# jnvance/DMRG.x

Measured on AMD Instinct MI355X. Metric: superblock MatMults/sec inside the ground-state eigensolve (Lanczos step = 1 MatMult + reorthogonalisation), higher is better.
Workload: dtype f64

## Files before the change

### dmrg.x_amd/csrc/eigs.hip

```cpp
#include "common.h"
#include <mutex>
#include <algorithm>
#include <chrono>
#include <cmath>
#include <cstring>
#include <cstddef>

namespace dmrgx {
namespace {

constexpr int DOT_BLOCKS = 1024, DOT_THREADS = 256, DOT_CHUNK = 8, MAX_NCV = 64, FUSE_NV = 24, GD_NV = 8;

__device__ __forceinline__ double wave_sum(double v) {
#pragma unroll
    for (int o = 32; o > 0; o >>= 1) v += __shfl_down(v, o, 64);
    return v;
}

template <bool VEC2>
__global__ void __launch_bounds__(DOT_THREADS)
multi_dot_kernel(const double* __restrict__ V, int64_t ldv, int nv, const double* __restrict__ w, int64_t n, double* __restrict__ partial)
{
    __shared__ double red[DOT_THREADS / 64][DOT_CHUNK];
    const int v0 = blockIdx.y * DOT_CHUNK;
    double acc[DOT_CHUNK];
#pragma unroll
    for (int i = 0; i < DOT_CHUNK; ++i) acc[i] = 0.0;
    if (VEC2) {
        const double2* __restrict__ w2 = reinterpret_cast<const double2*>(w);
        for (int64_t e = (int64_t)blockIdx.x * DOT_THREADS + threadIdx.x; e < n / 2; e += (int64_t)gridDim.x * DOT_THREADS) {
            const double2 wv = w2[e];
#pragma unroll
            for (int i = 0; i < DOT_CHUNK; ++i) {
                const int v = v0 + i;
                if (v < nv) { const double2 x = reinterpret_cast<const double2*>(V + (int64_t)v * ldv)[e]; acc[i] += x.x * wv.x + x.y * wv.y; }
                else if (v == nv) acc[i] += wv.x * wv.x + wv.y * wv.y;
            }
        }
    } else {
        for (int64_t e = (int64_t)blockIdx.x * DOT_THREADS + threadIdx.x; e < n; e += (int64_t)gridDim.x * DOT_THREADS) {
            const double wv = w[e];
#pragma unroll
            for (int i = 0; i < DOT_CHUNK; ++i) {
                const int v = v0 + i;
                if (v < nv) acc[i] += V[(int64_t)v * ldv + e] * wv;
                else if (v == nv) acc[i] += wv * wv;
            }
        }
    }
    const int lane = threadIdx.x & 63, wave = threadIdx.x >> 6;
#pragma unroll
    for (int i = 0; i < DOT_CHUNK; ++i) {
        const double s = wave_sum(acc[i]);
        if (lane == 0) red[wave][i] = s;
    }
    __syncthreads();
    if (threadIdx.x < DOT_CHUNK) {
        double s = 0.0;
        for (int wv = 0; wv < DOT_THREADS / 64; ++wv) s += red[wv][threadIdx.x];
        partial[(int64_t)(v0 + threadIdx.x) * gridDim.x + blockIdx.x] = s;
    }
}

__global__ void __launch_bounds__(DOT_THREADS)
reduce_partials_kernel(const double* __restrict__ partial, double* __restrict__ out, int count, int nblk)
{
    __shared__ double red[DOT_THREADS / 64];
    const int i = blockIdx.x;
    if (i >= count) return;
    double s = 0.0;
    for (int b = threadIdx.x; b < nblk; b += DOT_THREADS) s += partial[(int64_t)i * nblk + b];
    s = wave_sum(s);
    if ((threadIdx.x & 63) == 0) red[threadIdx.x >> 6] = s;
    __syncthreads();
    if (threadIdx.x == 0) { double t = 0.0; for (int k = 0; k < DOT_THREADS / 64; ++k) t += red[k]; out[i] = t; }
}

__global__ void __launch_bounds__(DOT_THREADS)
multi_axpy_kernel(const double* __restrict__ V, int64_t ldv, int nv, const double* __restrict__ c, double* __restrict__ w, int64_t n,
                  double* __restrict__ partial, double* __restrict__ hacc)
{
    __shared__ double cs[MAX_NCV + 1];
    __shared__ double red[DOT_THREADS / 64];
    if (threadIdx.x < nv) cs[threadIdx.x] = c[threadIdx.x];
    __syncthreads();
    if (blockIdx.x == 0 && threadIdx.x < nv && hacc) hacc[threadIdx.x] += cs[threadIdx.x];
    double nrm = 0.0;
    for (int64_t e = (int64_t)blockIdx.x * DOT_THREADS + threadIdx.x; e < n; e += (int64_t)gridDim.x * DOT_THREADS) {
        double x = w[e];
        for (int i = 0; i < nv; ++i) x -= cs[i] * V[(int64_t)i * ldv + e];
        w[e] = x;
        nrm += x * x;
    }
    nrm = wave_sum(nrm);
    if ((threadIdx.x & 63) == 0) red[threadIdx.x >> 6] = nrm;
    __syncthreads();
    if (threadIdx.x == 0) { double t = 0.0; for (int k = 0; k < DOT_THREADS / 64; ++k) t += red[k]; partial[blockIdx.x] = t; }
}

template <int NVMAX>
__global__ void __launch_bounds__(DOT_THREADS)
axpy_dot_kernel(const double* __restrict__ V, int64_t ldv, int nv, const double* __restrict__ c, double* __restrict__ w, int64_t n,
                double* __restrict__ partial, double* __restrict__ hacc)
{
    __shared__ double cs[NVMAX];
    __shared__ double red[DOT_THREADS / 64][NVMAX + 1];
    if (threadIdx.x < nv) cs[threadIdx.x] = c[threadIdx.x];
    __syncthreads();
    if (blockIdx.x == 0 && threadIdx.x < nv && hacc) hacc[threadIdx.x] += cs[threadIdx.x];
    double acc[NVMAX + 1];
#pragma unroll
    for (int i = 0; i <= NVMAX; ++i) acc[i] = 0.0;
    for (int64_t e = (int64_t)blockIdx.x * DOT_THREADS + threadIdx.x; e < n; e += (int64_t)gridDim.x * DOT_THREADS) {
        double v[NVMAX];
#pragma unroll
        for (int i = 0; i < NVMAX; ++i) v[i] = i < nv ? V[(int64_t)i * ldv + e] : 0.0;
        double x = w[e];
#pragma unroll
        for (int i = 0; i < NVMAX; ++i) if (i < nv) x -= cs[i] * v[i];
        w[e] = x;
#pragma unroll
        for (int i = 0; i < NVMAX; ++i) if (i < nv) acc[i] += v[i] * x;
        acc[NVMAX] += x * x;
    }
    const int lane = threadIdx.x & 63, wave = threadIdx.x >> 6;
#pragma unroll
    for (int i = 0; i <= NVMAX; ++i) {
        if (i < nv || i == NVMAX) {
            const double s2 = wave_sum(acc[i]);
            if (lane == 0) red[wave][i] = s2;
        }
    }
    __syncthreads();
    if (threadIdx.x <= nv) {
        const int src = threadIdx.x < nv ? threadIdx.x : NVMAX;
        double s2 = 0.0;
        for (int wv = 0; wv < DOT_THREADS / 64; ++wv) s2 += red[wv][src];
        partial[(int64_t)threadIdx.x * gridDim.x + blockIdx.x] = s2;
    }
}

template <bool VEC2>
__global__ void __launch_bounds__(DOT_THREADS)
axpy_normalise_kernel(const double* __restrict__ V, int64_t ldv, int nv, const double* __restrict__ c, const double* __restrict__ w,
                      double* __restrict__ dst, int64_t n, double* __restrict__ beta2_out, double* __restrict__ hacc)
{
    __shared__ double cs[MAX_NCV + 2];
    if (threadIdx.x <= nv) cs[threadIdx.x] = c[threadIdx.x];
    __syncthreads();
    if (blockIdx.x == 0 && threadIdx.x < nv && hacc) hacc[threadIdx.x] += cs[threadIdx.x];
    double s2 = cs[nv], sc = 0.0;
    for (int i = 0; i < nv; ++i) { s2 -= cs[i] * cs[i]; sc += cs[i] * cs[i]; }
    s2 = s2 > 0.0 ? s2 : 0.0;
    if (blockIdx.x == 0 && threadIdx.x == 0 && beta2_out) *beta2_out = s2;
    const double inv = s2 > 1e-290 ? 1.0 / sqrt(s2) : 0.0;
    if (sc <= 1e-27 * cs[nv]) nv = 0;
    if (VEC2) {
        const double2* __restrict__ w2 = reinterpret_cast<const double2*>(w);
        double2* __restrict__ d2 = reinterpret_cast<double2*>(dst);
        for (int64_t e = (int64_t)blockIdx.x * DOT_THREADS + threadIdx.x; e < n / 2; e += (int64_t)gridDim.x * DOT_THREADS) {
            double2 x = w2[e];
            for (int i = 0; i < nv; ++i) { const double2 v = reinterpret_cast<const double2*>(V + (int64_t)i * ldv)[e]; x.x -= cs[i] * v.x; x.y -= cs[i] * v.y; }
            x.x *= inv; x.y *= inv;
            d2[e] = x;
        }
    } else {
        for (int64_t e = (int64_t)blockIdx.x * DOT_THREADS + threadIdx.x; e < n; e += (int64_t)gridDim.x * DOT_THREADS) {
            double x = w[e];
            for (int i = 0; i < nv; ++i) x -= cs[i] * V[(int64_t)i * ldv + e];
            dst[e] = x * inv;
        }
    }
}

__global__ void norm_after_projection_kernel(const double* __restrict__ c, int nv, double* __restrict__ nrm2)
{
    if (threadIdx.x == 0 && blockIdx.x == 0) { double s = c[nv]; for (int i = 0; i < nv; ++i) s -= c[i] * c[i]; *nrm2 = s > 0.0 ? s : 0.0; }
}

__global__ void scale_copy_kernel(const double* __restrict__ src, double* __restrict__ dst, int64_t n, const double* __restrict__ nrm2)
{
    const double s2 = *nrm2;
    const double inv = s2 > 1e-290 ? 1.0 / sqrt(s2) : 0.0;
    for (int64_t e = (int64_t)blockIdx.x * blockDim.x + threadIdx.x; e < n; e += (int64_t)gridDim.x * blockDim.x) dst[e] = src[e] * inv;
}

__global__ void __launch_bounds__(DOT_THREADS)
basis_rotate_kernel(const double* __restrict__ V, int64_t ldv, int m, const double* __restrict__ Q, int ldq, int k,
                    double* __restrict__ out, int64_t ldo, int64_t n)
{
    __shared__ double qs[MAX_NCV * DOT_CHUNK];
    const int j0 = blockIdx.y * DOT_CHUNK;
    for (int t = threadIdx.x; t < m * DOT_CHUNK; t += DOT_THREADS) {
        const int i = t / DOT_CHUNK, j = t % DOT_CHUNK;
        qs[t] = (j0 + j < k) ? Q[i * ldq + j0 + j] : 0.0;
    }
    __syncthreads();
    for (int64_t e = (int64_t)blockIdx.x * DOT_THREADS + threadIdx.x; e < n; e += (int64_t)gridDim.x * DOT_THREADS) {
        double acc[DOT_CHUNK];
#pragma unroll
        for (int j = 0; j < DOT_CHUNK; ++j) acc[j] = 0.0;
        for (int i = 0; i < m; ++i) {
            const double v = V[(int64_t)i * ldv + e];
#pragma unroll
            for (int j = 0; j < DOT_CHUNK; ++j) acc[j] += v * qs[i * DOT_CHUNK + j];
        }
#pragma unroll
        for (int j = 0; j < DOT_CHUNK; ++j) if (j0 + j < k) out[(int64_t)(j0 + j) * ldo + e] = acc[j];
    }
}

constexpr int GD_MAX = FUSE_NV;
constexpr int GD_LD = GD_MAX;
struct GdState {
    double G[GD_MAX * GD_LD];
    double Y[GD_MAX * GD_LD];
    double th[GD_MAX];
    double y[GD_MAX];
    double yprev[GD_MAX];
    double Q[GD_MAX * GD_LD];
    double theta;
    double hv0_2;
    double e0[GD_MAX];
    int after_restart;
    int pad_;
};

constexpr int RITZ_THREADS = 64;
__global__ void __launch_bounds__(RITZ_THREADS)
gd_ritz_kernel(GdState* __restrict__ S, const double* __restrict__ col_src, int col_is_partial, int nblk, int mm, int warm, int restart, int keep)
{
    __shared__ double A[GD_MAX][GD_MAX + 1], Qa[GD_MAX][GD_MAX + 1], Yn[GD_MAX][GD_MAX + 1], Yp[GD_MAX][GD_MAX + 1];
    __shared__ double col[GD_MAX + 1], cs_c[GD_MAX / 2], cs_s[GD_MAX / 2], dg[GD_MAX], thp[GD_MAX], ths[GD_MAX];
    __shared__ int pp[GD_MAX / 2], qq[GD_MAX / 2], perm[GD_MAX];
    __shared__ double offn, dgn;
    const int tid = threadIdx.x, lane = tid;
    const int j = mm - 1;
    if (warm && mm > 1) {
        for (int e = tid; e < (mm - 1) * (mm - 1); e += RITZ_THREADS) Yp[e / (mm - 1)][e % (mm - 1)] = S->Y[(e / (mm - 1)) * GD_LD + e % (mm - 1)];
        if (tid < mm - 1) thp[tid] = S->th[tid];
    }
    const double yold = tid < GD_MAX ? S->y[tid] : 0.0;
    const int was_restart = S->after_restart;
// ... 346 lines not shown
    static thread_local double* p = nullptr;
    if (!p && hipHostMalloc((void**)&p, (8 + MAX_NCV + 2) * sizeof(double), hipHostMallocDefault) != hipSuccess) { (void)hipGetLastError(); p = nullptr; }
    return p;
}
static bool start_too_light(const dmrgx_eigs_opts* opts, const double* pin)
{
    return opts->min_initial_norm2 > 0.0 && pin && !(pin[2] >= opts->min_initial_norm2);
}

extern "C" dmrgx_status dmrgx_eigs_lowest(dmrgx_kron_plan* plan, const dmrgx_eigs_opts* opts, double* e0,
                                          double* psi_full, dmrgx_eigs_stats* stats, void* stream)
{
    hipStream_t st = (hipStream_t)stream;
    if (!plan || !opts || !e0 || !psi_full) DMRGX_FAIL(DMRGX_ERR_ARG, "eigs_lowest: null argument");
    dmrgx_kron_info I;
    DMRGX_CHK(dmrgx_kron_plan_info(plan, &I));
    const bool gd_space = std::min<int64_t>(opts->ncv > 0 ? opts->ncv : 16, I.n_states) >= 2;
    if (opts->method == 1 && opts->use_initial && opts->max_matvec <= 0 && gd_space) return eigs_davidson(plan, opts, e0, psi_full, stats, st);
    const bool dist = I.vec_len != I.n_states;
    const bool hooks = opts->allgather && opts->allreduce_sum;
    if (dist && !hooks && !opts->comm) DMRGX_FAIL(DMRGX_ERR_ARG, "eigs_lowest: a striped plan needs a communicator (opts->comm) or the allgather/allreduce hooks");
    auto gather_full = [&](double* full) -> dmrgx_status {
        return hooks ? opts->allgather(opts->user, full, I.seg_stride, st) : dmrgx_comm_allgather(opts->comm, full, I.seg_stride, st);
    };
    const int64_t n = I.local_len, N = I.n_states;
    int m = opts->ncv > 0 ? opts->ncv : 16;
    m = (int)std::min<int64_t>(std::min(m, MAX_NCV), N);
    m = (int)std::max<int64_t>(m, std::min<int64_t>(2, N));
    if (m < 1) DMRGX_FAIL(DMRGX_ERR_ARG, "eigs_lowest: empty problem");
    const int max_it = opts->max_it > 0 ? opts->max_it : std::max<int>(100, (int)(2 * N / m));
    const double tol = opts->tol > 0 ? opts->tol : 1e-8;
    const auto t_begin = std::chrono::steady_clock::now();

    DevBuf dV, dW, dX, dTmp, dPartial, dScal, dQ;
    DMRGX_CHK(dV.alloc_f64((size_t)(m + 1) * n, st));
    DMRGX_CHK(dW.alloc_f64((size_t)n, st));
    DMRGX_CHK(dTmp.alloc_f64((size_t)(m / 2 + 2) * n, st));
    if (dist) DMRGX_CHK(dX.alloc_f64((size_t)I.vec_len, st));
    DMRGX_CHK(dPartial.alloc_f64((size_t)(MAX_NCV + DOT_CHUNK + 1) * DOT_BLOCKS, st));
    const int row = m + 2;
    DMRGX_CHK(dScal.alloc_f64((size_t)((m + 1) * row + 3 * (MAX_NCV + 2)), st));
    DMRGX_CHK(dQ.alloc_f64((size_t)MAX_NCV * MAX_NCV, st));
    double* V = dV.as<double>();
    double* w = dW.as<double>();
    double* c1 = dScal.as<double>() + (size_t)(m + 1) * row;
    double* c2 = c1 + (MAX_NCV + 2);
    double* nrm = c2 + (MAX_NCV + 2);
    auto Hrow = [&](int j) { return dScal.as<double>() + (size_t)j * row; };
    auto vec = [&](int j) { return V + (size_t)j * n; };
    DMRGX_HIP(zero_async(dV.p, dV.bytes, st));
    DMRGX_HIP(zero_async(dW.p, dW.bytes, st));
    if (dist) DMRGX_HIP(zero_async(dX.p, dX.bytes, st));

    const bool vec2 = (n % 2 == 0);
    const int nblk = DOT_BLOCKS;
    auto allreduce = [&](double* buf, int64_t count) -> dmrgx_status {
        if (!dist) return DMRGX_OK;
        return hooks ? opts->allreduce_sum(opts->user, buf, count, st) : dmrgx_comm_allreduce_sum(opts->comm, buf, count, st);
    };
    auto multi_dot = [&](int nv) -> dmrgx_status {
        const int chunks = (nv + 1 + DOT_CHUNK - 1) / DOT_CHUNK;
        if (vec2) hipLaunchKernelGGL(multi_dot_kernel<true>, dim3(nblk, chunks), dim3(DOT_THREADS), 0, st, V, n, nv, w, n, dPartial.as<double>());
        else hipLaunchKernelGGL(multi_dot_kernel<false>, dim3(nblk, chunks), dim3(DOT_THREADS), 0, st, V, n, nv, w, n, dPartial.as<double>());
        DMRGX_HIP(hipGetLastError());
        hipLaunchKernelGGL(reduce_partials_kernel, dim3(nv + 1), dim3(DOT_THREADS), 0, st, dPartial.as<double>(), c1, nv + 1, nblk);
        DMRGX_HIP(hipGetLastError());
        return allreduce(c1, nv + 1);
    };
    auto multi_axpy = [&](int nv, double* hacc, bool final) -> dmrgx_status {
        if (final) { hipLaunchKernelGGL(norm_after_projection_kernel, dim3(1), dim3(64), 0, st, c1, nv, nrm); DMRGX_HIP(hipGetLastError()); }
        hipLaunchKernelGGL(multi_axpy_kernel, dim3(nblk), dim3(DOT_THREADS), 0, st, V, n, nv, c1, w, n, dPartial.as<double>(), hacc);
        DMRGX_HIP(hipGetLastError());
        return DMRGX_OK;
    };
    auto normalise_into = [&](double* dst) -> dmrgx_status {
        hipLaunchKernelGGL(scale_copy_kernel, dim3(1024), dim3(256), 0, st, w, dst, n, nrm);
        DMRGX_HIP(hipGetLastError());
        return DMRGX_OK;
    };
    CommTimer ctimer(st);
    auto matvec = [&](const double* v_local, double* y_local) -> dmrgx_status {
        if (!dist) return dmrgx_kron_apply(plan, v_local, y_local, st);
        DMRGX_HIP(hipMemcpyAsync(dX.as<double>() + I.local_offset, v_local, (size_t)n * sizeof(double), hipMemcpyDeviceToDevice, st));
        ctimer.mark();
        DMRGX_CHK(gather_full(dX.as<double>()));
        ctimer.mark();
        const dmrgx_status rc = dmrgx_kron_apply(plan, dX.as<double>(), y_local, st);
        ctimer.mark();
        return rc;
    };

    if (opts->use_initial) DMRGX_HIP(hipMemcpyAsync(w, psi_full + I.local_offset, (size_t)n * sizeof(double), hipMemcpyDeviceToDevice, st));
    else {
        if (!dist) { hipLaunchKernelGGL(random_fill_kernel, dim3(1024), dim3(256), 0, st, w, n, opts->seed, (int64_t)0); DMRGX_HIP(hipGetLastError()); }
        else {
            DevBuf ref;
            DMRGX_CHK(ref.alloc((size_t)N * sizeof(double)));
            hipLaunchKernelGGL(random_fill_kernel, dim3(1024), dim3(256), 0, st, ref.as<double>(), N, opts->seed, (int64_t)0);
            DMRGX_HIP(hipGetLastError());
            DMRGX_CHK(dmrgx_kron_vec_to_striped(plan, ref.as<double>(), dX.as<double>(), st));
            DMRGX_HIP(hipMemcpyAsync(w, dX.as<double>() + I.local_offset, (size_t)n * sizeof(double), hipMemcpyDeviceToDevice, st));
            DMRGX_HIP(hipStreamSynchronize(st));
        }
    }
// ... 10 lines not shown
    if (looks && !look_buf) {
        DMRGX_HIP(hipHostMalloc((void**)&look_buf, 2 * look_stride * sizeof(double), hipHostMallocDefault));
        DMRGX_HIP(hipEventCreateWithFlags(&look_ev[0], hipEventDisableTiming)); DMRGX_HIP(hipEventCreateWithFlags(&look_ev[1], hipEventDisableTiming));
    }
    int look_mm[2] = {0, 0};
    std::vector<double> T((size_t)m * m, 0.0), theta, Q, hbuf((size_t)(m + 1) * row);
    int k = 0, n_matvec = 0, restarts = 0, converged = 0;
    double beta_m = 0.0, resid = 0.0, lambda = 0.0;
    std::vector<double> Qdev;
    auto null_start = [&]() { return opts->use_initial && restarts == 0 && k == 0 && ((!(std::fabs(hbuf[0]) > 0.0) && !(hbuf[(size_t)m + 1] > 0.0)) || start_too_light(opts, pin)); };
    auto redo_from_random = [&]() -> dmrgx_status {
        dV.release(); dW.release(); dTmp.release(); dX.release();
        dmrgx_eigs_opts o2 = *opts;
        o2.use_initial = 0;
        dmrgx_eigs_stats s2;
        memset(&s2, 0, sizeof(s2));
        const dmrgx_status rc = dmrgx_eigs_lowest(plan, &o2, e0, psi_full, &s2, (void*)st);
        if (stats) { *stats = s2; stats->n_matvec += n_matvec; stats->start_rejected = 1;
                     stats->seconds = std::chrono::duration<double>(std::chrono::steady_clock::now() - t_begin).count(); }
        return rc;
    };
    while (true) {
        DMRGX_HIP(zero_async(Hrow(k), (size_t)(m + 1 - k) * row * sizeof(double), st));
        int jend = m;
        if (opts->max_matvec > 0) jend = std::min(m, k + std::max(0, opts->max_matvec - n_matvec));
        const bool capped = jend < m || (opts->max_matvec > 0 && n_matvec + (m - k) >= opts->max_matvec);
        bool early = false;
        for (int j = k; j < jend; ++j) {
            DMRGX_CHK(matvec(vec(j), w));
            ++n_matvec;
            const int nv = j + 1;
            DMRGX_CHK(multi_dot(nv));
            if (nv <= FUSE_NV) {
                hipLaunchKernelGGL(axpy_dot_kernel<FUSE_NV>, dim3(nblk), dim3(DOT_THREADS), 0, st, V, n, nv, c1, w, n, dPartial.as<double>(), Hrow(j));
                DMRGX_HIP(hipGetLastError());
                hipLaunchKernelGGL(reduce_partials_kernel, dim3(nv + 1), dim3(DOT_THREADS), 0, st, dPartial.as<double>(), c2, nv + 1, nblk);
                DMRGX_HIP(hipGetLastError());
                DMRGX_CHK(allreduce(c2, nv + 1));
            } else {
                DMRGX_CHK(multi_axpy(nv, Hrow(j), false));
                DMRGX_CHK(multi_dot(nv));
                DMRGX_HIP(hipMemcpyAsync(c2, c1, (size_t)(nv + 1) * sizeof(double), hipMemcpyDeviceToDevice, st));
            }
            if (vec2) hipLaunchKernelGGL(axpy_normalise_kernel<true>, dim3(nblk), dim3(DOT_THREADS), 0, st, V, n, nv, c2, w, vec(j + 1), n, Hrow(j) + m + 1, Hrow(j));
            else hipLaunchKernelGGL(axpy_normalise_kernel<false>, dim3(nblk), dim3(DOT_THREADS), 0, st, V, n, nv, c2, w, vec(j + 1), n, Hrow(j) + m + 1, Hrow(j));
            DMRGX_HIP(hipGetLastError());
            if (looks && j + 1 < m) {
                const int slot = j & 1;
                DMRGX_HIP(hipMemcpyAsync(look_buf + (size_t)slot * look_stride, dScal.p, (size_t)(m + 1) * row * sizeof(double), hipMemcpyDeviceToHost, st));
                DMRGX_HIP(hipEventRecord(look_ev[slot], st));
                look_mm[slot] = j + 1;
            }
            if (looks && j > k && look_mm[(j - 1) & 1] == j) {
                const int slot = (j - 1) & 1;
                look_mm[slot] = 0;
                DMRGX_HIP(hipEventSynchronize(look_ev[slot]));
                std::copy(look_buf + (size_t)slot * look_stride, look_buf + (size_t)slot * look_stride + (size_t)(m + 1) * row, hbuf.begin());
                if (null_start()) { DMRGX_HIP(hipStreamSynchronize(st)); return redo_from_random(); }
                const int mm = j;
                std::vector<double> A((size_t)mm * mm, 0.0), th, Qs;
                for (int jj = 0; jj < mm; ++jj) for (int i = 0; i <= jj; ++i) {
                    const double v = (jj >= k) ? hbuf[(size_t)jj * row + i] : T[(size_t)i * m + jj];
                    A[(size_t)i * mm + jj] = v; A[(size_t)jj * mm + i] = v;
                }
                jacobi_eigh(mm, A, th, Qs);
                const double r = std::fabs(std::sqrt(std::max(0.0, hbuf[(size_t)(mm - 1) * row + m + 1])) * Qs[(size_t)(mm - 1) * mm + 0]);
                static const bool trace = getenv("DMRGX_EIGS_TRACE") != nullptr;
                if (trace) fprintf(stderr, "[eigs] look at matvec %d (queued: %d): theta %.12f  |r| %.3e  (target %.3e)\n", n_matvec - 1, n_matvec, th[0], r, tol * std::fabs(th[0]));
                if (r <= tol * std::max(std::fabs(th[0]), 1e-300)) { jend = j + 1; early = true; break; }
            }
        }
        look_mm[0] = look_mm[1] = 0;
        DMRGX_HIP(hipMemcpyAsync(hbuf.data(), dScal.p, (size_t)(m + 1) * row * sizeof(double), hipMemcpyDeviceToHost, st));
        DMRGX_HIP(hipStreamSynchronize(st));
        if (null_start()) return redo_from_random();
        if (jend < m) {
            const int mm = jend;
            if (mm < 1) break;
            std::vector<double> A((size_t)mm * mm, 0.0), th, Qs;
            for (int j = 0; j < mm; ++j) for (int i = 0; i <= j; ++i) {
                const double v = (j >= k) ? hbuf[(size_t)j * row + i] : T[(size_t)i * m + j];
                A[(size_t)i * mm + j] = v; A[(size_t)j * mm + i] = v;
            }
            jacobi_eigh(mm, A, th, Qs);
            lambda = th[0];
            resid = std::fabs(std::sqrt(std::max(0.0, hbuf[(size_t)(mm - 1) * row + m + 1])) * Qs[(size_t)(mm - 1) * mm + 0]);
            Q.assign((size_t)m * m, 0.0);
            for (int i = 0; i < mm; ++i) Q[(size_t)i * m + 0] = Qs[(size_t)i * mm + 0];
            ++restarts;
            if (early) converged = 1;
            break;
        }
        for (int j = k; j < m; ++j)
            for (int i = 0; i <= j; ++i) { T[(size_t)i * m + j] = hbuf[(size_t)j * row + i]; T[(size_t)j * m + i] = T[(size_t)i * m + j]; }
        beta_m = std::sqrt(std::max(0.0, hbuf[(size_t)(m - 1) * row + m + 1]));
        std::vector<double> A = T;
        jacobi_eigh(m, A, theta, Q);
        lambda = theta[0];
        resid = std::fabs(beta_m * Q[(size_t)(m - 1) * m + 0]);
        ++restarts;
        if (resid <= tol * std::max(std::fabs(lambda), 1e-300) || m == N) { converged = 1; break; }
        if (restarts >= max_it || capped) break;
        const int kk = std::max(1, std::min(m / 2, m - 1));
        Qdev.assign((size_t)m * kk, 0.0);
        for (int i = 0; i < m; ++i) for (int j = 0; j < kk; ++j) Qdev[(size_t)i * kk + j] = Q[(size_t)i * m + j];
        DMRGX_HIP(h2d_async(dQ.p, Qdev.data(), Qdev.size() * sizeof(double), st));
        hipLaunchKernelGGL(basis_rotate_kernel, dim3(1024, (kk + DOT_CHUNK - 1) / DOT_CHUNK), dim3(DOT_THREADS), 0, st,
                           V, n, m, dQ.as<double>(), kk, kk, dTmp.as<double>(), n, n);
        DMRGX_HIP(hipGetLastError());
        DMRGX_HIP(hipMemcpyAsync(V, dTmp.p, (size_t)kk * n * sizeof(double), hipMemcpyDeviceToDevice, st));
        DMRGX_HIP(hipMemcpyAsync(vec(kk), vec(m), (size_t)n * sizeof(double), hipMemcpyDeviceToDevice, st));
        DMRGX_HIP(hipStreamSynchronize(st));
        std::fill(T.begin(), T.end(), 0.0);
        for (int i = 0; i < kk; ++i) T[(size_t)i * m + i] = theta[i];
        k = kk;
    }
    Qdev.assign((size_t)m, 0.0);
    for (int i = 0; i < m; ++i) Qdev[i] = Q[(size_t)i * m + 0];
    DMRGX_HIP(h2d_async(dQ.p, Qdev.data(), Qdev.size() * sizeof(double), st));
    hipLaunchKernelGGL(basis_rotate_kernel, dim3(1024, 1), dim3(DOT_THREADS), 0, st, V, n, m, dQ.as<double>(), 1, 1, w, n, n);
    DMRGX_HIP(hipGetLastError());
    DMRGX_CHK(multi_dot(0));
    DMRGX_HIP(hipMemcpyAsync(nrm, c1, sizeof(double), hipMemcpyDeviceToDevice, st));
    if (!dist) DMRGX_CHK(normalise_into(psi_full));
    else {
        DMRGX_CHK(normalise_into(psi_full + I.local_offset));
        DMRGX_CHK(gather_full(psi_full));
    }
    DMRGX_HIP(hipStreamSynchronize(st));
    *e0 = lambda;
    if (stats) {
        stats->n_matvec = n_matvec; stats->n_restart = restarts; stats->converged = converged; stats->start_rejected = 0; stats->residual = resid;
        stats->seconds = std::chrono::duration<double>(std::chrono::steady_clock::now() - t_begin).count();
    }
    if (!converged) DMRGX_FAIL(DMRGX_ERR_NOTCONV, "eigs_lowest: not converged after %d restarts (residual %.3e)", restarts, resid);
    return DMRGX_OK;
}


static dmrgx_status eigs_davidson(dmrgx_kron_plan* plan, const dmrgx_eigs_opts* opts, double* e0, double* psi_full, dmrgx_eigs_stats* stats, hipStream_t st)
{
    dmrgx_kron_info I;
    DMRGX_CHK(dmrgx_kron_plan_info(plan, &I));
    const bool dist = I.vec_len != I.n_states;
    const bool hooks = opts->allgather && opts->allreduce_sum;
    if (dist && !hooks && !opts->comm) DMRGX_FAIL(DMRGX_ERR_ARG, "eigs_lowest: a striped plan needs a communicator (opts->comm) or the allgather/allreduce hooks");
    const int64_t n = I.local_len, N = I.n_states;
    const int64_t ld = (n + 1) & ~(int64_t)1;
    int m = opts->ncv > 0 ? opts->ncv : GD_NV;
    m = (int)std::min<int64_t>(std::min(m, GD_MAX - 1), N);
    if (m < 2) DMRGX_FAIL(DMRGX_ERR_ARG, "eigs_lowest (gd): needs at least a two-dimensional search space");
    if (m < 3 && N >= 3) m = 3;
    const int keep = std::max(1, std::min(opts->gd_minv > 0 ? opts->gd_minv : 1, m - 2));
// ... 23 lines not shown
    DMRGX_CHK(dScal.alloc_f64((size_t)(3 * (MAX_NCV + 2)), st));
    DMRGX_CHK(dState.alloc(sizeof(GdState)));
    double* V = dV.as<double>();
    double* W = dW.as<double>();
    double* t = dT.as<double>();
    double* c1 = dScal.as<double>();
    double* c2 = c1 + (MAX_NCV + 2);
    double* nrm = c2 + (MAX_NCV + 2);
    GdState* S = dState.as<GdState>();
    const double* const S_y = (const double*)((const char*)dState.p + offsetof(GdState, y));
    const double* const S_e0 = (const double*)((const char*)dState.p + offsetof(GdState, e0));
    const double* const S_Q = (const double*)((const char*)dState.p + offsetof(GdState, Q));
    auto vec = [&](int j) { return V + (size_t)j * ld; };
    auto wvec = [&](int j) { return W + (size_t)j * ld; };
    if (dist) { DMRGX_HIP(zero_async(dV.p, dV.bytes, st)); DMRGX_HIP(zero_async(dW.p, dW.bytes, st)); }
    if (dist) DMRGX_HIP(zero_async(dT.p, dT.bytes, st));
    DMRGX_HIP(zero_async(dState.p, dState.bytes, st));
    if (dist) DMRGX_HIP(zero_async(dX.p, dX.bytes, st));
    mark("buffers");
    DMRGX_CHK(dmrgx_kron_diag(plan, dD.as<double>(), st));
    if (ld != n) {
        hipLaunchKernelGGL(gd_zero_pads_kernel, dim3(1), dim3(64), 0, st, W, ld, m + 1, n, t, dD.as<double>());
        DMRGX_HIP(hipGetLastError());
    }
    mark("diagonal");
    auto allreduce = [&](double* buf, int64_t count) -> dmrgx_status {
        if (!dist) return DMRGX_OK;
        return hooks ? opts->allreduce_sum(opts->user, buf, count, st) : dmrgx_comm_allreduce_sum(opts->comm, buf, count, st);
    };
    auto gather_full = [&](double* full) -> dmrgx_status {
        return hooks ? opts->allgather(opts->user, full, I.seg_stride, st) : dmrgx_comm_allgather(opts->comm, full, I.seg_stride, st);
    };
    auto multi_dot = [&](int nv, const double* x, double* out, bool reduce) -> dmrgx_status {
        const int chunks = (nv + 1 + DOT_CHUNK - 1) / DOT_CHUNK;
        hipLaunchKernelGGL(multi_dot_kernel<true>, dim3(nblk, chunks), dim3(DOT_THREADS), 0, st, V, ld, nv, x, ld, dPartial.as<double>());
        DMRGX_HIP(hipGetLastError());
        if (!reduce) return DMRGX_OK;
        hipLaunchKernelGGL(reduce_partials_kernel, dim3(nv + 1), dim3(DOT_THREADS), 0, st, dPartial.as<double>(), out, nv + 1, nblk);
        DMRGX_HIP(hipGetLastError());
        return allreduce(out, nv + 1);
    };
    auto orthonormalise_tail = [&](int nv, double* x, double* dst) -> dmrgx_status {
        if (nv <= GD_NV) hipLaunchKernelGGL(axpy_dot_kernel<GD_NV>, dim3(nblk), dim3(DOT_THREADS), 0, st, V, ld, nv, c1, x, ld, dPartial.as<double>(), (double*)nullptr);
        else hipLaunchKernelGGL(axpy_dot_kernel<FUSE_NV>, dim3(nblk), dim3(DOT_THREADS), 0, st, V, ld, nv, c1, x, ld, dPartial.as<double>(), (double*)nullptr);
        DMRGX_HIP(hipGetLastError());
        hipLaunchKernelGGL(reduce_partials_kernel, dim3(nv + 1), dim3(DOT_THREADS), 0, st, dPartial.as<double>(), c2, nv + 1, nblk);
        DMRGX_HIP(hipGetLastError());
        DMRGX_CHK(allreduce(c2, nv + 1));
        hipLaunchKernelGGL(axpy_normalise_kernel<true>, dim3(nblk), dim3(DOT_THREADS), 0, st, V, ld, nv, c2, x, dst, ld, (double*)nullptr, (double*)nullptr);
        DMRGX_HIP(hipGetLastError());
        return DMRGX_OK;
    };
    CommTimer ctimer(st);
    auto matvec = [&](const double* v_local, double* y_local) -> dmrgx_status {
        if (!dist) return dmrgx_kron_apply(plan, v_local, y_local, st);
        DMRGX_HIP(hipMemcpyAsync(dX.as<double>() + I.local_offset, v_local, (size_t)n * sizeof(double), hipMemcpyDeviceToDevice, st));
        ctimer.mark();
        DMRGX_CHK(gather_full(dX.as<double>()));
        ctimer.mark();
        const dmrgx_status rc = dmrgx_kron_apply(plan, dX.as<double>(), y_local, st);
        ctimer.mark();
        return rc;
    };

    if (opts->use_initial) DMRGX_HIP(hipMemcpyAsync(t, psi_full + I.local_offset, (size_t)n * sizeof(double), hipMemcpyDeviceToDevice, st));
    else if (!dist) { hipLaunchKernelGGL(random_fill_kernel, dim3(1024), dim3(256), 0, st, t, n, opts->seed, (int64_t)0); DMRGX_HIP(hipGetLastError()); }
    else {
        DevBuf ref;
        DMRGX_CHK(ref.alloc((size_t)N * sizeof(double)));
        hipLaunchKernelGGL(random_fill_kernel, dim3(1024), dim3(256), 0, st, ref.as<double>(), N, opts->seed, (int64_t)0);
        DMRGX_HIP(hipGetLastError());
        DMRGX_CHK(dmrgx_kron_vec_to_striped(plan, ref.as<double>(), dX.as<double>(), st));
        DMRGX_HIP(hipMemcpyAsync(t, dX.as<double>() + I.local_offset, (size_t)n * sizeof(double), hipMemcpyDeviceToDevice, st));
        DMRGX_HIP(hipStreamSynchronize(st));
    }
    DMRGX_CHK(multi_dot(0, t, c1, true));
    DMRGX_CHK(orthonormalise_tail(0, t, vec(0)));
    double* const pin = opts->use_initial ? pinned_scalars() : nullptr;
    if (pin) { pin[2] = 0.0; DMRGX_HIP(hipMemcpyAsync(pin + 2, c2, sizeof(double), hipMemcpyDeviceToHost, st)); }
    mark("start vector");

    static thread_local double* h_look = nullptr;
// ... 114 lines not shown
```

### dmrg.x_amd/csrc/kron_plan.hip

```cpp
#include "ggemm.h"
#include <algorithm>
#include <map>
#include <set>
#include <tuple>
#include <cstdlib>
#include <memory>
#include <new>

namespace dmrgx {

namespace {

struct NCell {
    int32_t q, r0, c0, nr, nc, kind;
    double scale;
    const double* data;
    int64_t ld;
    bool tr;
};

struct PCell {
    int32_t q, r0, c0, nr, nc, kind;
    double scale;
    int64_t off;
// ... 29 lines not shown
    double* dst = arena + k.dst_off;
    if (!k.tr) {
        for (int r = ty; r < 32; r += 8) {
            const int i = i0 + r, j = j0 + tx;
            if (i < k.nr && j < k.nc) { const double v = k.a * k.src[(size_t)i * k.lds + j]; double& o = dst[(size_t)i * k.ldd + j]; o = k.round == 0 ? v : o + v; }
        }
    } else {
        for (int r = ty; r < 32; r += 8) {
            const int j = j0 + r, i = i0 + tx;
            buf[r][tx] = (i < k.nr && j < k.nc) ? k.src[(size_t)j * k.lds + i] : 0.0;
        }
        __syncthreads();
        for (int r = ty; r < 32; r += 8) {
            const int i = i0 + r, j = j0 + tx;
            if (i < k.nr && j < k.nc) { const double v = k.a * buf[tx][r]; double& o = dst[(size_t)i * k.ldd + j]; o = k.round == 0 ? v : o + v; }
        }
    }
}

struct LayoutSeg { int64_t ref_off, full_off; int32_t nrow, ncol, ref_ld, full_ld; };
__global__ void layout_copy_kernel(const LayoutSeg* __restrict__ segs, const double* __restrict__ src, double* __restrict__ dst, int to_striped)
{
    const LayoutSeg s = segs[blockIdx.y];
    const int64_t n = (int64_t)s.nrow * s.ncol;
    for (int64_t e = (int64_t)blockIdx.x * blockDim.x + threadIdx.x; e < n; e += (int64_t)gridDim.x * blockDim.x) {
        const int64_t i = e / s.ncol, j = e % s.ncol;
        const int64_t a = s.ref_off + i * s.ref_ld + j, b = s.full_off + i * s.full_ld + j;
        if (to_striped) dst[b] = src[a]; else dst[a] = src[b];
    }
}

struct RedTask { int64_t dst_off, slab_off; int32_t ldc, M, N, nslab; };
struct RedTile { int32_t task, chunk; };
constexpr int RED_CHUNK = 2048;
__global__ __launch_bounds__(256) void slab_reduce_kernel(const RedTile* __restrict__ tiles, const RedTask* __restrict__ tasks,
                                                          double* __restrict__ y, const double* __restrict__ arena)
{
    const RedTile t = tiles[blockIdx.x];
    const RedTask k = tasks[t.task];
    const uint32_t mn = (uint32_t)k.M * (uint32_t)k.N, N = (uint32_t)k.N;
    const double* sl = arena + k.slab_off;
    double* yb = y + k.dst_off;
    constexpr int NE = RED_CHUNK / 256;
    const uint32_t e0 = (uint32_t)t.chunk * RED_CHUNK + threadIdx.x;
    double v[NE];
    double* d[NE];
#pragma unroll
    for (int i = 0; i < NE; ++i) {
        const uint32_t e = min(e0 + (uint32_t)i * 256u, mn - 1);
        const uint32_t row = e / N, col = e - row * N;
        d[i] = yb + (size_t)row * k.ldc + col;
        v[i] = *d[i];
    }
    for (int s = 0; s < k.nslab; ++s) {
        const double* p = sl + (size_t)s * mn;
#pragma unroll
        for (int i = 0; i < NE; ++i) v[i] += p[min(e0 + (uint32_t)i * 256u, mn - 1)];
    }
#pragma unroll
    for (int i = 0; i < NE; ++i) if (e0 + (uint32_t)i * 256u < mn) *d[i] = v[i];
}

struct DiagSrc { int64_t off; int32_t ld, n, round; int64_t dst; double scale; };
struct DiagSeg { int64_t out_off; int32_t nrow, ncol; int64_t l0, r0; };
__global__ void __launch_bounds__(256) diag_gather_kernel(const DiagSrc* __restrict__ src, int nsrc, int round, const double* __restrict__ arena, double* __restrict__ dvec)
{
    const int t = blockIdx.x;
    if (t >= nsrc) return;
    const DiagSrc s = src[t];
    if (s.round != round) return;
    for (int i = threadIdx.x; i < s.n; i += 256) dvec[s.dst + i] += s.off >= 0 ? arena[s.off + (int64_t)i * (s.ld + 1)] : s.scale;
}
__global__ void __launch_bounds__(256) diag_fill_kernel(const DiagSeg* __restrict__ segs, const double* __restrict__ dA, const double* __restrict__ dB,
                                                         int nterms, int64_t NL, int64_t NR, double* __restrict__ out)
{
    const DiagSeg s = segs[blockIdx.y];
    const int64_t n = (int64_t)s.nrow * s.ncol;
    for (int64_t e = (int64_t)blockIdx.x * 256 + threadIdx.x; e < n; e += (int64_t)gridDim.x * 256) {
        const int64_t l = e / s.ncol, r = e % s.ncol;
        double d = 0.0;
        for (int t = 0; t < nterms; ++t) d += dA[(int64_t)t * NL + s.l0 + l] * dB[(int64_t)t * NR + s.r0 + r];
        out[s.out_off + e] = d;
    }
}

}
}

using namespace dmrgx;

enum : int32_t { BASE_ARENA = 0, BASE_X = 1, BASE_Y = 2 };

namespace dmrgx {
// ... 1194 lines not shown
```

Measured before the change: 359.8.

## Widen multi-dot batching, pad basis stride, in-place restart, vectorised slab reduce

The multi-dot kernel now handles up to 24 basis vectors per block with batched double2 loads, so fewer passes over w are needed. The basis stride is padded to a multiple of 32 so vector loads are always legal. Small-m restarts rotate the basis in place instead of going through a temp buffer plus memcpy, and the host sync after restart is removed. Axpy-dot dispatch picks a smaller template for small nv and keeps coefficients in registers. The slab reduction in the Kronecker matvec uses double2 loads with batched slab prefetch when alignment allows. These changes add register pressure and rely on padding and alignment assumptions holding.

After: 363.3, median of 6. Within noise of the previous version (+1.0%).

```diff
diff --git a/dmrg.x_amd/csrc/eigs.hip b/dmrg.x_amd/csrc/eigs.hip
--- a/dmrg.x_amd/csrc/eigs.hip
+++ b/dmrg.x_amd/csrc/eigs.hip
@@ -10,6 +10,8 @@
 namespace {
 
 constexpr int DOT_BLOCKS = 1024, DOT_THREADS = 256, DOT_CHUNK = 8, MAX_NCV = 64, FUSE_NV = 24, GD_NV = 8;
+constexpr int DOT_BATCH = 8;
+constexpr int64_t DOT_ALIGN = 32;
 
 __device__ __forceinline__ double wave_sum(double v) {
 #pragma unroll
@@ -17,49 +19,62 @@
     return v;
 }
 
-template <bool VEC2>
+template <int NVMAX>
 __global__ void __launch_bounds__(DOT_THREADS)
 multi_dot_kernel(const double* __restrict__ V, int64_t ldv, int nv, const double* __restrict__ w, int64_t n, double* __restrict__ partial)
 {
-    __shared__ double red[DOT_THREADS / 64][DOT_CHUNK];
-    const int v0 = blockIdx.y * DOT_CHUNK;
-    double acc[DOT_CHUNK];
-#pragma unroll
-    for (int i = 0; i < DOT_CHUNK; ++i) acc[i] = 0.0;
-    if (VEC2) {
-        const double2* __restrict__ w2 = reinterpret_cast<const double2*>(w);
-        for (int64_t e = (int64_t)blockIdx.x * DOT_THREADS + threadIdx.x; e < n / 2; e += (int64_t)gridDim.x * DOT_THREADS) {
-            const double2 wv = w2[e];
-#pragma unroll
-            for (int i = 0; i < DOT_CHUNK; ++i) {
-                const int v = v0 + i;
-                if (v < nv) { const double2 x = reinterpret_cast<const double2*>(V + (int64_t)v * ldv)[e]; acc[i] += x.x * wv.x + x.y * wv.y; }
-                else if (v == nv) acc[i] += wv.x * wv.x + wv.y * wv.y;
-            }
-        }
-    } else {
-        for (int64_t e = (int64_t)blockIdx.x * DOT_THREADS + threadIdx.x; e < n; e += (int64_t)gridDim.x * DOT_THREADS) {
-            const double wv = w[e];
-#pragma unroll
-            for (int i = 0; i < DOT_CHUNK; ++i) {
-                const int v = v0 + i;
-                if (v < nv) acc[i] += V[(int64_t)v * ldv + e] * wv;
-                else if (v == nv) acc[i] += wv * wv;
-            }
-        }
+    static_assert(NVMAX % DOT_BATCH == 0, "rows are loaded DOT_BATCH at a time");
+    __shared__ double red[DOT_THREADS / 64][NVMAX + 1];
+    const int v0 = blockIdx.y * NVMAX;
+    const int cnt = min(NVMAX, nv - v0);
+    const double* __restrict__ Vb = V + (int64_t)v0 * ldv;
+    double acc[NVMAX + 1];
+#pragma unroll
+    for (int i = 0; i <= NVMAX; ++i) acc[i] = 0.0;
+    const int64_t tid = (int64_t)blockIdx.x * DOT_THREADS + threadIdx.x, stride = (int64_t)gridDim.x * DOT_THREADS;
+    const double2* __restrict__ w2 = reinterpret_cast<const double2*>(w);
+    for (int64_t e = tid; e < n / 2; e += stride) {
+        const double2 wv = w2[e];
+#pragma unroll
+        for (int b = 0; b < NVMAX; b += DOT_BATCH) {
+            if (b < cnt) {
+                double2 x[DOT_BATCH];
+#pragma unroll
+                for (int i = 0; i < DOT_BATCH; ++i) x[i] = b + i < cnt ? reinterpret_cast<const double2*>(Vb + (int64_t)(b + i) * ldv)[e] : make_double2(0.0, 0.0);
+#pragma unroll
+                for (int i = 0; i < DOT_BATCH; ++i) acc[b + i] += x[i].x * wv.x + x[i].y * wv.y;
+            }
+        }
+        acc[NVMAX] += wv.x * wv.x + wv.y * wv.y;
+    }
+    if ((n & 1) && tid == 0) {
+        const double wv = w[n - 1];
+#pragma unroll
+        for (int i = 0; i < NVMAX; ++i) if (i < cnt) acc[i] += Vb[(int64_t)i * ldv + n - 1] * wv;
+        acc[NVMAX] += wv * wv;
     }
     const int lane = threadIdx.x & 63, wave = threadIdx.x >> 6;
 #pragma unroll
-    for (int i = 0; i < DOT_CHUNK; ++i) {
-        const double s = wave_sum(acc[i]);
-        if (lane == 0) red[wave][i] = s;
-    }
-    __syncthreads();
-    if (threadIdx.x < DOT_CHUNK) {
+    for (int i = 0; i <= NVMAX; ++i) {
+        if (i < cnt || i == NVMAX) {
+            const double s = wave_sum(acc[i]);
+            if (lane == 0) red[wave][i] = s;
+        }
+    }
+    __syncthreads();
+    if ((int)threadIdx.x < cnt || ((int)threadIdx.x == max(cnt, 0) && blockIdx.y == 0)) {
+        const bool ww = (int)threadIdx.x >= cnt;
+        const int src = ww ? NVMAX : (int)threadIdx.x;
         double s = 0.0;
-        for (int wv = 0; wv < DOT_THREADS / 64; ++wv) s += red[wv][threadIdx.x];
-        partial[(int64_t)(v0 + threadIdx.x) * gridDim.x + blockIdx.x] = s;
-    }
+        for (int wv = 0; wv < DOT_THREADS / 64; ++wv) s += red[wv][src];
+        partial[(int64_t)(ww ? nv : v0 + (int)threadIdx.x) * gridDim.x + blockIdx.x] = s;
+    }
+}
+static void launch_multi_dot(const double* V, int64_t ldv, int nv, const double* w, int64_t n, double* partial, int nblk, hipStream_t st)
+{
+    if (nv <= 8) hipLaunchKernelGGL(multi_dot_kernel<8>, dim3(nblk, 1), dim3(DOT_THREADS), 0, st, V, ldv, nv, w, n, partial);
+    else if (nv <= 16) hipLaunchKernelGGL(multi_dot_kernel<16>, dim3(nblk, 1), dim3(DOT_THREADS), 0, st, V, ldv, nv, w, n, partial);
+    else hipLaunchKernelGGL(multi_dot_kernel<FUSE_NV>, dim3(nblk, (nv + FUSE_NV - 1) / FUSE_NV), dim3(DOT_THREADS), 0, st, V, ldv, nv, w, n, partial);
 }
 
 __global__ void __launch_bounds__(DOT_THREADS)
@@ -103,11 +118,11 @@
 axpy_dot_kernel(const double* __restrict__ V, int64_t ldv, int nv, const double* __restrict__ c, double* __restrict__ w, int64_t n,
                 double* __restrict__ partial, double* __restrict__ hacc)
 {
-    __shared__ double cs[NVMAX];
     __shared__ double red[DOT_THREADS / 64][NVMAX + 1];
-    if (threadIdx.x < nv) cs[threadIdx.x] = c[threadIdx.x];
-    __syncthreads();
-    if (blockIdx.x == 0 && threadIdx.x < nv && hacc) hacc[threadIdx.x] += cs[threadIdx.x];
+    double cs[NVMAX];
+#pragma unroll
+    for (int i = 0; i < NVMAX; ++i) cs[i] = i < nv ? c[i] : 0.0;
+    if (blockIdx.x == 0 && threadIdx.x < nv && hacc) hacc[threadIdx.x] += c[threadIdx.x];
     double acc[NVMAX + 1];
 #pragma unroll
     for (int i = 0; i <= NVMAX; ++i) acc[i] = 0.0;
@@ -139,8 +154,13 @@
         partial[(int64_t)threadIdx.x * gridDim.x + blockIdx.x] = s2;
     }
 }
-
-template <bool VEC2>
+static void launch_axpy_dot(const double* V, int64_t ldv, int nv, const double* c, double* w, int64_t n, double* partial, double* hacc, int nblk, hipStream_t st)
+{
+    if (nv <= GD_NV) hipLaunchKernelGGL(axpy_dot_kernel<GD_NV>, dim3(nblk), dim3(DOT_THREADS), 0, st, V, ldv, nv, c, w, n, partial, hacc);
+    else if (nv <= 16) hipLaunchKernelGGL(axpy_dot_kernel<16>, dim3(nblk), dim3(DOT_THREADS), 0, st, V, ldv, nv, c, w, n, partial, hacc);
+    else hipLaunchKernelGGL(axpy_dot_kernel<FUSE_NV>, dim3(nblk), dim3(DOT_THREADS), 0, st, V, ldv, nv, c, w, n, partial, hacc);
+}
+
 __global__ void __launch_bounds__(DOT_THREADS)
 axpy_normalise_kernel(const double* __restrict__ V, int64_t ldv, int nv, const double* __restrict__ c, const double* __restrict__ w,
                       double* __restrict__ dst, int64_t n, double* __restrict__ beta2_out, double* __restrict__ hacc)
@@ -155,21 +175,19 @@
     if (blockIdx.x == 0 && threadIdx.x == 0 && beta2_out) *beta2_out = s2;
     const double inv = s2 > 1e-290 ? 1.0 / sqrt(s2) : 0.0;
     if (sc <= 1e-27 * cs[nv]) nv = 0;
-    if (VEC2) {
-        const double2* __restrict__ w2 = reinterpret_cast<const double2*>(w);
-        double2* __restrict__ d2 = reinterpret_cast<double2*>(dst);
-        for (int64_t e = (int64_t)blockIdx.x * DOT_THREADS + threadIdx.x; e < n / 2; e += (int64_t)gridDim.x * DOT_THREADS) {
-            double2 x = w2[e];
-            for (int i = 0; i < nv; ++i) { const double2 v = reinterpret_cast<const double2*>(V + (int64_t)i * ldv)[e]; x.x -= cs[i] * v.x; x.y -= cs[i] * v.y; }
-            x.x *= inv; x.y *= inv;
-            d2[e] = x;
-        }
-    } else {
-        for (int64_t e = (int64_t)blockIdx.x * DOT_THREADS + threadIdx.x; e < n; e += (int64_t)gridDim.x * DOT_THREADS) {
-            double x = w[e];
-            for (int i = 0; i < nv; ++i) x -= cs[i] * V[(int64_t)i * ldv + e];
-            dst[e] = x * inv;
-        }
+    const int64_t tid = (int64_t)blockIdx.x * DOT_THREADS + threadIdx.x;
+    const double2* __restrict__ w2 = reinterpret_cast<const double2*>(w);
+    double2* __restrict__ d2 = reinterpret_cast<double2*>(dst);
+    for (int64_t e = tid; e < n / 2; e += (int64_t)gridDim.x * DOT_THREADS) {
+        double2 x = w2[e];
+        for (int i = 0; i < nv; ++i) { const double2 v = reinterpret_cast<const double2*>(V + (int64_t)i * ldv)[e]; x.x -= cs[i] * v.x; x.y -= cs[i] * v.y; }
+        x.x *= inv; x.y *= inv;
+        d2[e] = x;
+    }
+    if ((n & 1) && tid == 0) {
+        double x = w[n - 1];
+        for (int i = 0; i < nv; ++i) x -= cs[i] * V[(int64_t)i * ldv + n - 1];
+        dst[n - 1] = x * inv;
     }
 }
 
@@ -209,6 +227,48 @@
         for (int j = 0; j < DOT_CHUNK; ++j) if (j0 + j < k) out[(int64_t)(j0 + j) * ldo + e] = acc[j];
     }
 }
+
+template <int M, int W>
+__global__ void __launch_bounds__(DOT_THREADS)
+restart_inplace_kernel(double* V, int64_t ldv, int m, const double* __restrict__ Q, int kk, int64_t n)
+{
+    __shared__ double qs[M * M];
+    for (int t = threadIdx.x; t < m * kk; t += DOT_THREADS) qs[t] = Q[t];
+    __syncthreads();
+    const int64_t tid = (int64_t)blockIdx.x * DOT_THREADS + threadIdx.x, stride = (int64_t)gridDim.x * DOT_THREADS;
+    auto single = [&](int64_t e) {
+        double v[M];
+#pragma unroll
+        for (int i = 0; i < M; ++i) v[i] = i < m ? V[(int64_t)i * ldv + e] : 0.0;
+        const double r = V[(int64_t)m * ldv + e];
+        for (int j = 0; j < kk; ++j) {
+            double a = 0.0;
+#pragma unroll
+            for (int i = 0; i < M; ++i) if (i < m) a += v[i] * qs[i * kk + j];
+            V[(int64_t)j * ldv + e] = a;
+        }
+        V[(int64_t)kk * ldv + e] = r;
+    };
+    if (W == 2) {
+        for (int64_t e = tid; e < n / 2; e += stride) {
+            double2 v[M];
+#pragma unroll
+            for (int i = 0; i < M; ++i) v[i] = i < m ? reinterpret_cast<const double2*>(V + (int64_t)i * ldv)[e] : make_double2(0.0, 0.0);
+            const double2 r = reinterpret_cast<const double2*>(V + (int64_t)m * ldv)[e];
+            for (int j = 0; j < kk; ++j) {
+                double2 a = make_double2(0.0, 0.0);
+#pragma unroll
+                for (int i = 0; i < M; ++i) if (i < m) { const double q = qs[i * kk + j]; a.x += v[i].x * q; a.y += v[i].y * q; }
+                reinterpret_cast<double2*>(V + (int64_t)j * ldv)[e] = a;
+            }
+            reinterpret_cast<double2*>(V + (int64_t)kk * ldv)[e] = r;
+        }
+        if ((n & 1) && tid == 0) single(n - 1);
+    } else {
+        for (int64_t e = tid; e < n; e += stride) single(e);
+    }
+}
+constexpr int RESTART_INPLACE_MAX = 32;
 
 constexpr int GD_MAX = FUSE_NV;
 constexpr int GD_LD = GD_MAX;
@@ -621,10 +681,11 @@
     const double tol = opts->tol > 0 ? opts->tol : 1e-8;
     const auto t_begin = std::chrono::steady_clock::now();
 
+    const int64_t ldv = (n + DOT_ALIGN - 1) / DOT_ALIGN * DOT_ALIGN;
     DevBuf dV, dW, dX, dTmp, dPartial, dScal, dQ;
-    DMRGX_CHK(dV.alloc_f64((size_t)(m + 1) * n, st));
-    DMRGX_CHK(dW.alloc_f64((size_t)n, st));
-    DMRGX_CHK(dTmp.alloc_f64((size_t)(m / 2 + 2) * n, st));
+    DMRGX_CHK(dV.alloc_f64((size_t)(m + 1) * ldv, st));
+    DMRGX_CHK(dW.alloc_f64((size_t)ldv, st));
+    if (m > RESTART_INPLACE_MAX) { DMRGX_CHK(dTmp.alloc_f64((size_t)(m / 2 + 2) * ldv, st)); DMRGX_HIP(zero_async(dTmp.p, dTmp.bytes, st)); }
     if (dist) DMRGX_CHK(dX.alloc_f64((size_t)I.vec_len, st));
     DMRGX_CHK(dPartial.alloc_f64((size_t)(MAX_NCV + DOT_CHUNK + 1) * DOT_BLOCKS, st));
     const int row = m + 2;
@@ -636,21 +697,18 @@
     double* c2 = c1 + (MAX_NCV + 2);
     double* nrm = c2 + (MAX_NCV + 2);
     auto Hrow = [&](int j) { return dScal.as<double>() + (size_t)j * row; };
-    auto vec = [&](int j) { return V + (size_t)j * n; };
+    auto vec = [&](int j) { return V + (size_t)j * ldv; };
     DMRGX_HIP(zero_async(dV.p, dV.bytes, st));
     DMRGX_HIP(zero_async(dW.p, dW.bytes, st));
     if (dist) DMRGX_HIP(zero_async(dX.p, dX.bytes, st));
 
-    const bool vec2 = (n % 2 == 0);
     const int nblk = DOT_BLOCKS;
     auto allreduce = [&](double* buf, int64_t count) -> dmrgx_status {
         if (!dist) return DMRGX_OK;
         return hooks ? opts->allreduce_sum(opts->user, buf, count, st) : dmrgx_comm_allreduce_sum(opts->comm, buf, count, st);
     };
     auto multi_dot = [&](int nv) -> dmrgx_status {
-        const int chunks = (nv + 1 + DOT_CHUNK - 1) / DOT_CHUNK;
-        if (vec2) hipLaunchKernelGGL(multi_dot_kernel<true>, dim3(nblk, chunks), dim3(DOT_THREADS), 0, st, V, n, nv, w, n, dPartial.as<double>());
-        else hipLaunchKernelGGL(multi_dot_kernel<false>, dim3(nblk, chunks), dim3(DOT_THREADS), 0, st, V, n, nv, w, n, dPartial.as<double>());
+        launch_multi_dot(V, ldv, nv, w, n, dPartial.as<double>(), nblk, st);
         DMRGX_HIP(hipGetLastError());
         hipLaunchKernelGGL(reduce_partials_kernel, dim3(nv + 1), dim3(DOT_THREADS), 0, st, dPartial.as<double>(), c1, nv + 1, nblk);
         DMRGX_HIP(hipGetLastError());
@@ -658,7 +716,7 @@
     };
     auto multi_axpy = [&](int nv, double* hacc, bool final) -> dmrgx_status {
         if (final) { hipLaunchKernelGGL(norm_after_projection_kernel, dim3(1), dim3(64), 0, st, c1, nv, nrm); DMRGX_HIP(hipGetLastError()); }
-        hipLaunchKernelGGL(multi_axpy_kernel, dim3(nblk), dim3(DOT_THREADS), 0, st, V, n, nv, c1, w, n, dPartial.as<double>(), hacc);
+        hipLaunchKernelGGL(multi_axpy_kernel, dim3(nblk), dim3(DOT_THREADS), 0, st, V, ldv, nv, c1, w, n, dPartial.as<double>(), hacc);
         DMRGX_HIP(hipGetLastError());
         return DMRGX_OK;
     };
@@ -735,7 +793,7 @@
             const int nv = j + 1;
             DMRGX_CHK(multi_dot(nv));
             if (nv <= FUSE_NV) {
-                hipLaunchKernelGGL(axpy_dot_kernel<FUSE_NV>, dim3(nblk), dim3(DOT_THREADS), 0, st, V, n, nv, c1, w, n, dPartial.as<double>(), Hrow(j));
+                launch_axpy_dot(V, ldv, nv, c1, w, n, dPartial.as<double>(), Hrow(j), nblk, st);
                 DMRGX_HIP(hipGetLastError());
                 hipLaunchKernelGGL(reduce_partials_kernel, dim3(nv + 1), dim3(DOT_THREADS), 0, st, dPartial.as<double>(), c2, nv + 1, nblk);
                 DMRGX_HIP(hipGetLastError());
@@ -745,8 +803,7 @@
                 DMRGX_CHK(multi_dot(nv));
                 DMRGX_HIP(hipMemcpyAsync(c2, c1, (size_t)(nv + 1) * sizeof(double), hipMemcpyDeviceToDevice, st));
             }
-            if (vec2) hipLaunchKernelGGL(axpy_normalise_kernel<true>, dim3(nblk), dim3(DOT_THREADS), 0, st, V, n, nv, c2, w, vec(j + 1), n, Hrow(j) + m + 1, Hrow(j));
-            else hipLaunchKernelGGL(axpy_normalise_kernel<false>, dim3(nblk), dim3(DOT_THREADS), 0, st, V, n, nv, c2, w, vec(j + 1), n, Hrow(j) + m + 1, Hrow(j));
+            hipLaunchKernelGGL(axpy_normalise_kernel, dim3(nblk), dim3(DOT_THREADS), 0, st, V, ldv, nv, c2, w, vec(j + 1), n, Hrow(j) + m + 1, Hrow(j));
             DMRGX_HIP(hipGetLastError());
             if (looks && j + 1 < m) {
                 const int slot = j & 1;
@@ -808,12 +865,16 @@
         Qdev.assign((size_t)m * kk, 0.0);
         for (int i = 0; i < m; ++i) for (int j = 0; j < kk; ++j) Qdev[(size_t)i * kk + j] = Q[(size_t)i * m + j];
         DMRGX_HIP(h2d_async(dQ.p, Qdev.data(), Qdev.size() * sizeof(double), st));
-        hipLaunchKernelGGL(basis_rotate_kernel, dim3(1024, (kk + DOT_CHUNK - 1) / DOT_CHUNK), dim3(DOT_THREADS), 0, st,
-                           V, n, m, dQ.as<double>(), kk, kk, dTmp.as<double>(), n, n);
-        DMRGX_HIP(hipGetLastError());
-        DMRGX_HIP(hipMemcpyAsync(V, dTmp.p, (size_t)kk * n * sizeof(double), hipMemcpyDeviceToDevice, st));
-        DMRGX_HIP(hipMemcpyAsync(vec(kk), vec(m), (size_t)n * sizeof(double), hipMemcpyDeviceToDevice, st));
-        DMRGX_HIP(hipStreamSynchronize(st));
+        if (m <= 16) hipLaunchKernelGGL((restart_inplace_kernel<16, 2>), dim3(nblk), dim3(DOT_THREADS), 0, st, V, ldv, m, dQ.as<double>(), kk, n);
+        else if (m <= RESTART_INPLACE_MAX) hipLaunchKernelGGL((restart_inplace_kernel<RESTART_INPLACE_MAX, 1>), dim3(nblk), dim3(DOT_THREADS), 0, st, V, ldv, m, dQ.as<double>(), kk, n);
+        else {
+            hipLaunchKernelGGL(basis_rotate_kernel, dim3(1024, (kk + DOT_CHUNK - 1) / DOT_CHUNK), dim3(DOT_THREADS), 0, st,
+                               V, ldv, m, dQ.as<double>(), kk, kk, dTmp.as<double>(), ldv, n);
+            DMRGX_HIP(hipGetLastError());
+            DMRGX_HIP(hipMemcpyAsync(V, dTmp.p, (size_t)kk * ldv * sizeof(double), hipMemcpyDeviceToDevice, st));
+            DMRGX_HIP(hipMemcpyAsync(vec(kk), vec(m), (size_t)n * sizeof(double), hipMemcpyDeviceToDevice, st));
+        }
+        DMRGX_HIP(hipGetLastError());
         std::fill(T.begin(), T.end(), 0.0);
         for (int i = 0; i < kk; ++i) T[(size_t)i * m + i] = theta[i];
         k = kk;
@@ -821,7 +882,7 @@
     Qdev.assign((size_t)m, 0.0);
     for (int i = 0; i < m; ++i) Qdev[i] = Q[(size_t)i * m + 0];
     DMRGX_HIP(h2d_async(dQ.p, Qdev.data(), Qdev.size() * sizeof(double), st));
-    hipLaunchKernelGGL(basis_rotate_kernel, dim3(1024, 1), dim3(DOT_THREADS), 0, st, V, n, m, dQ.as<double>(), 1, 1, w, n, n);
+    hipLaunchKernelGGL(basis_rotate_kernel, dim3(1024, 1), dim3(DOT_THREADS), 0, st, V, ldv, m, dQ.as<double>(), 1, 1, w, ldv, n);
     DMRGX_HIP(hipGetLastError());
     DMRGX_CHK(multi_dot(0));
     DMRGX_HIP(hipMemcpyAsync(nrm, c1, sizeof(double), hipMemcpyDeviceToDevice, st));
@@ -911,8 +972,7 @@
         return hooks ? opts->allgather(opts->user, full, I.seg_stride, st) : dmrgx_comm_allgather(opts->comm, full, I.seg_stride, st);
     };
     auto multi_dot = [&](int nv, const double* x, double* out, bool reduce) -> dmrgx_status {
-        const int chunks = (nv + 1 + DOT_CHUNK - 1) / DOT_CHUNK;
-        hipLaunchKernelGGL(multi_dot_kernel<true>, dim3(nblk, chunks), dim3(DOT_THREADS), 0, st, V, ld, nv, x, ld, dPartial.as<double>());
+        launch_multi_dot(V, ld, nv, x, ld, dPartial.as<double>(), nblk, st);
         DMRGX_HIP(hipGetLastError());
         if (!reduce) return DMRGX_OK;
         hipLaunchKernelGGL(reduce_partials_kernel, dim3(nv + 1), dim3(DOT_THREADS), 0, st, dPartial.as<double>(), out, nv + 1, nblk);
@@ -920,13 +980,12 @@
         return allreduce(out, nv + 1);
     };
     auto orthonormalise_tail = [&](int nv, double* x, double* dst) -> dmrgx_status {
-        if (nv <= GD_NV) hipLaunchKernelGGL(axpy_dot_kernel<GD_NV>, dim3(nblk), dim3(DOT_THREADS), 0, st, V, ld, nv, c1, x, ld, dPartial.as<double>(), (double*)nullptr);
-        else hipLaunchKernelGGL(axpy_dot_kernel<FUSE_NV>, dim3(nblk), dim3(DOT_THREADS), 0, st, V, ld, nv, c1, x, ld, dPartial.as<double>(), (double*)nullptr);
+        launch_axpy_dot(V, ld, nv, c1, x, ld, dPartial.as<double>(), (double*)nullptr, nblk, st);
         DMRGX_HIP(hipGetLastError());
         hipLaunchKernelGGL(reduce_partials_kernel, dim3(nv + 1), dim3(DOT_THREADS), 0, st, dPartial.as<double>(), c2, nv + 1, nblk);
         DMRGX_HIP(hipGetLastError());
         DMRGX_CHK(allreduce(c2, nv + 1));
-        hipLaunchKernelGGL(axpy_normalise_kernel<true>, dim3(nblk), dim3(DOT_THREADS), 0, st, V, ld, nv, c2, x, dst, ld, (double*)nullptr, (double*)nullptr);
+        hipLaunchKernelGGL(axpy_normalise_kernel, dim3(nblk), dim3(DOT_THREADS), 0, st, V, ld, nv, c2, x, dst, ld, (double*)nullptr, (double*)nullptr);
         DMRGX_HIP(hipGetLastError());
         return DMRGX_OK;
     };
diff --git a/dmrg.x_amd/csrc/kron_plan.hip b/dmrg.x_amd/csrc/kron_plan.hip
--- a/dmrg.x_amd/csrc/kron_plan.hip
+++ b/dmrg.x_amd/csrc/kron_plan.hip
@@ -85,33 +85,60 @@
 
 struct RedTask { int64_t dst_off, slab_off; int32_t ldc, M, N, nslab; };
 struct RedTile { int32_t task, chunk; };
-constexpr int RED_CHUNK = 2048;
+constexpr int RED_CHUNK = 1024, RED_SLABS = 8;
+__device__ __forceinline__ void red_add(double& a, double b) { a += b; }
+__device__ __forceinline__ void red_add(double2& a, const double2& b) { a.x += b.x; a.y += b.y; }
+template <int W, class T>
+__device__ __forceinline__ void slab_reduce_chunk(const RedTask& k, uint32_t chunk, double* __restrict__ yb, const double* __restrict__ sl)
+{
+    constexpr int NI = RED_CHUNK / 256 / W;
+    const uint32_t mn = (uint32_t)k.M * (uint32_t)k.N, N = (uint32_t)k.N;
+    const uint32_t step = 256u * W, step_r = step / N, step_c = step - step_r * N;
+    uint32_t e = chunk * RED_CHUNK + threadIdx.x * W;
+    uint32_t row = e / N, col = e - row * N;
+    uint32_t se[NI];
+    size_t ye[NI];
+    bool ok[NI];
+#pragma unroll
+    for (int i = 0; i < NI; ++i) {
+        ok[i] = e < mn;
+        se[i] = ok[i] ? e : 0u;
+        ye[i] = ok[i] ? (size_t)row * k.ldc + col : (size_t)0;
+        e += step; row += step_r; col += step_c;
+        if (col >= N) { col -= N; ++row; }
+    }
+    T v[NI];
+#pragma unroll
+    for (int i = 0; i < NI; ++i) v[i] = *reinterpret_cast<const T*>(yb + ye[i]);
+    for (int s0 = 0; s0 < k.nslab; s0 += RED_SLABS) {
+        T t[RED_SLABS][NI];
+#pragma unroll
+        for (int b = 0; b < RED_SLABS; ++b) {
+            if (s0 + b < k.nslab) {
+                const double* __restrict__ p = sl + (size_t)(s0 + b) * mn;
+#pragma unroll
+                for (int i = 0; i < NI; ++i) t[b][i] = *reinterpret_cast<const T*>(p + se[i]);
+            }
+        }
+#pragma unroll
+        for (int b = 0; b < RED_SLABS; ++b) {
+            if (s0 + b < k.nslab) {
+#pragma unroll
+                for (int i = 0; i < NI; ++i) red_add(v[i], t[b][i]);
+            }
+        }
+    }
+#pragma unroll
+    for (int i = 0; i < NI; ++i) if (ok[i]) *reinterpret_cast<T*>(yb + ye[i]) = v[i];
+}
 __global__ __launch_bounds__(256) void slab_reduce_kernel(const RedTile* __restrict__ tiles, const RedTask* __restrict__ tasks,
                                                           double* __restrict__ y, const double* __restrict__ arena)
 {
     const RedTile t = tiles[blockIdx.x];
     const RedTask k = tasks[t.task];
-    const uint32_t mn = (uint32_t)k.M * (uint32_t)k.N, N = (uint32_t)k.N;
-    const double* sl = arena + k.slab_off;
-    double* yb = y + k.dst_off;
-    constexpr int NE = RED_CHUNK / 256;
-    const uint32_t e0 = (uint32_t)t.chunk * RED_CHUNK + threadIdx.x;
-    double v[NE];
-    double* d[NE];
-#pragma unroll
-    for (int i = 0; i < NE; ++i) {
-        const uint32_t e = min(e0 + (uint32_t)i * 256u, mn - 1);
-        const uint32_t row = e / N, col = e - row * N;
-        d[i] = yb + (size_t)row * k.ldc + col;
-        v[i] = *d[i];
-    }
-    for (int s = 0; s < k.nslab; ++s) {
-        const double* p = sl + (size_t)s * mn;
-#pragma unroll
-        for (int i = 0; i < NE; ++i) v[i] += p[min(e0 + (uint32_t)i * 256u, mn - 1)];
-    }
-#pragma unroll
-    for (int i = 0; i < NE; ++i) if (e0 + (uint32_t)i * 256u < mn) *d[i] = v[i];
+    const bool pairs = (((uint32_t)k.N | (uint32_t)k.ldc | (uint32_t)k.dst_off | (uint32_t)k.slab_off) & 1u) == 0 && ((((uintptr_t)y) | ((uintptr_t)arena)) & 15) == 0;
+    if (pairs) slab_reduce_chunk<2, double2>(k, (uint32_t)t.chunk, y + k.dst_off, arena + k.slab_off);
+    else slab_reduce_chunk<1, double>(k, (uint32_t)t.chunk, y + k.dst_off, arena + k.slab_off);
 }
 
 struct DiagSrc { int64_t off; int32_t ld, n, round; int64_t dst; double scale; };
```
